# JuliaGaussianProcesses/ApproximateGPs.jl

Hardware: AMD Instinct MI355X
Metric: SVGP ELBO evals/sec at N=1e6, M=1024 (higher is better)
Workload: dtype f64

## Files before the change

### approximategps.jl_amd/csrc/api.hip

```cpp
#include <hip/hip_runtime.h>

#include <algorithm>
#include <functional>
#include <memory>
#include <cmath>
#include <cstdio>
#include <cstddef>
#include <cstdlib>
#include <cstring>
#include <new>
#include <string>
#include <vector>

#include "../../include/svgp_mi355x.h"
#include "ctx.hpp"
#include "kernels.hpp"
#include "knobs.hpp"
#include "lik.hpp"

using namespace svgp;

inline unsigned event_flags(bool timing) {
  static const bool fence = exp_int("SVGP_EVENT_FENCE", 0) == 1;
  return (timing ? 0u : unsigned(hipEventDisableTiming)) | (fence ? 0u : unsigned(hipEventDisableSystemFence));
// ... 136 lines not shown
    m->gh_w.release();
    m->gh_n = 0;
    if (gh > 0) {
      std::vector<double> xs(gh), ws(gh);
      if (gauss_hermite(gh, xs.data(), ws.data()) != SVGP_OK) return fail(ctx, SVGP_INVALID_ARG, "Gauss-Hermite rule failed to converge");
      for (auto& w : ws) w /= 1.7724538509055160273;
      hipError_t e = m->gh_x.alloc(gh * 8);
      if (e == hipSuccess) e = m->gh_w.alloc(gh * 8);
      if (e == hipSuccess) e = hipMemcpy(m->gh_x.p, xs.data(), gh * 8, hipMemcpyHostToDevice);
      if (e == hipSuccess) e = hipMemcpy(m->gh_w.p, ws.data(), gh * 8, hipMemcpyHostToDevice);
      if (e != hipSuccess) {
        m->gh_x.release();
        m->gh_w.release();
        return fail(ctx, e == hipErrorOutOfMemory ? SVGP_OOM : SVGP_HIP_ERROR, std::string("upload of the Gauss-Hermite rule: ") + hipGetErrorString(e));
      }
    }
    m->gh_n = gh;
  }
  HIPC(ctx, hipStreamSynchronize(ctx->stream));
  m->prepared = false;
  return SVGP_OK;
}

KernelParams kparams(const svgp_model* m) {
  KernelParams kp;
  kp.family = m->desc.kernel;
  kp.d = m->d;
  kp.variance = m->desc.variance;
  kp.invl = m->invl.p;
  return kp;
}

inline size_t info_bytes(int64_t Mp) { return (sizeof(int) * size_t(1 + 2 * (Mp / 128)) + 255) / 256 * 256; }
int ensure_overlap(svgp_ctx* ctx, size_t state_doubles);
int enqueue_prep(svgp_ctx* ctx, svgp_model* m, bool overlap = false, const RowHook* hook = nullptr) {
  hipStream_t s = ctx->stream;
  const KernelParams kp = kparams(m);
  HIPC(ctx, hipMemsetAsync(m->info.as<int>(), 0, info_bytes(m->Mp), s));
  launch_scale_inputs(m->dtype, s, m->z_raw.p, m->desc.layout_z, m->d, m->M, m->Mp, m->invl.p, m->zs.p);
  KCHECK(ctx, "scale_inputs");
  if (overlap) {
    launch_pack_q(m->dtype, s, m->Lq_raw.p, m->m_raw.p, m->M, m->Mp, m->U.p, m->mp.p);
    KCHECK(ctx, "pack_q");
    HIPC(ctx, hipEventRecord(ctx->ev_fork, s));
    TREC(ctx, ctx->ev_ov[0], s);
    if (hook && hook->fn) hook->fn(hook->user, -1);
  }
  launch_kuu(m->dtype, s, kp, m->zs.p, m->M, m->Mp, m->desc.jitter, m->L.p);
  KCHECK(ctx, "kuu");
  TREC(ctx, ctx->ev_chol[0], s);
  hipEvent_t rows[16] = {};
  if (overlap) std::copy(std::begin(ctx->ev_row), std::end(ctx->ev_row), rows);
  launch_potrf(m->dtype, s, m->L.p, m->T.p, m->Mp, m->info.as<int>(), reinterpret_cast<unsigned*>(m->info.as<int>() + 1), ctx->num_cus, overlap ? rows : nullptr,
               overlap ? hook : nullptr);
  KCHECK(ctx, "potrf");
  TREC(ctx, ctx->ev_chol[1], s);
  if (overlap) {
    launch_kl_terms(m->dtype, s, m->Lq_raw.p, m->m_raw.p, m->L.p, m->M, m->Mp, m->scal.as<double>());
  } else if (m->desc.parametrization == SVGP_NONCENTERED) {
    launch_pack_q(m->dtype, s, m->Lq_raw.p, m->m_raw.p, m->M, m->Mp, m->U.p, m->mp.p);
    launch_kl_terms(m->dtype, s, m->Lq_raw.p, m->m_raw.p, m->L.p, m->M, m->Mp, m->scal.as<double>());
  } else {
    launch_pad_lower(m->dtype, s, m->Lq_raw.p, m->M, m->Mp, m->B.p);
// ... 77 lines not shown
  int64_t lda = 0;
  bool skip_expect = false;
  const void* mux = nullptr;
};

int enqueue_strips(svgp_ctx* ctx, svgp_model* m, const void* x, int64_t ldx, const void* y, int64_t off, int64_t len,
                   const StripOuts& o) {
  StripPlan plan = strip_plan(m->dtype, m->Mp, len, ctx->num_cus);
  if (plan.concurrent_tail && (o.A || o.C || o.At || o.Ct)) plan = strip_plan_single(m->dtype, m->Mp, len, ctx->num_cus);
  const size_t wb_main = plan.grid ? strip_work_bytes(m->dtype, m->Mp, plan.nt, plan.grid) : 0;
  const size_t wb_tail = plan.nt_tail ? strip_work_bytes(m->dtype, m->Mp, plan.nt_tail, plan.grid_tail) : 0;
  int rc = ensure_scratch(ctx, plan.concurrent_tail ? wb_main : (wb_main > wb_tail ? wb_main : wb_tail), size_t(len));
  if (rc) return rc;
  if (plan.concurrent_tail) {
    rc = ensure_stream2(ctx);
    if (rc) return rc;
    rc = ctx->work2.reserve(ctx, wb_tail, "the concurrent tail's scratch");
    if (rc) return rc;
  }
  StripArgs a{};
  a.T = m->T.p;
  a.U = m->U.p;
  a.zs = m->zs.p;
  a.mp = m->mp.p;
  a.x = x;
  a.work = ctx->work.p;
  a.counter = ctx->counter.as<unsigned>();
  a.mom_mu = ctx->mom_mu();
  a.mom_var = ctx->mom_var();
  a.A_out = o.A;
  a.C_out = o.C;
  a.At_out = o.At;
  a.Ct_out = o.Ct;
  a.lda = o.lda;
  a.ldx = ldx;
  a.off = off;
  a.len = len;
  a.Mp = m->Mp;
  a.M = m->M;
  a.kp = kparams(m);
  a.mean_const = m->desc.mean_const;
  a.mux = o.mux;
  LikParams lp{};
  lp.lik = m->desc.likelihood;
  lp.gh_n = m->gh_n;
  lp.sigma2 = lik_param(m->desc);
// ... 101 lines not shown
  KCHECK(ctx, "strip (segmented: panel)");
  if (I == 0) TREC(ctx, ctx->ev_ov[1], s2);
  if (I == 1 && r.pre) {
    const int rcp = (*r.pre)();
    if (rcp) return rcp;
  }
  return SVGP_OK;
}

void seg_row_hook(void* user, int row) {
  SegRun& r = *static_cast<SegRun*>(user);
  if (r.rc == SVGP_OK) r.rc = seg_enqueue_row(r, row);
}

int seg_prepare_forward(svgp_ctx* ctx, svgp_model* m, const void* x, int64_t ldx, int64_t off, int64_t len, const OverlapPlan& op, SegRun& r) {
  const int nP = int(m->Mp / 128);
  const size_t wb1 = strip_work_bytes(m->dtype, m->Mp, op.nt, int(op.nstrips)), wb = wb1;
  int rc = ctx->work_seg.reserve(ctx, wb, "the segmented strips' scratch");
  if (rc == SVGP_OK) rc = ensure_scratch(ctx, 0, size_t(len));
  if (rc) return rc;
  r.ctx = ctx; r.m = m; r.op = op; r.grad = false; r.nP = nP; r.wb1 = wb1;
  r.split = seg_split_factor(ctx, nP, op.nstrips);
  StripArgs& a = r.a;
  a.T = m->T.p; a.U = m->U.p; a.zs = m->zs.p; a.mp = m->mp.p; a.x = x; a.work = ctx->work_seg.p; a.counter = ctx->counter2.as<unsigned>();
  a.mom_mu = ctx->mom_mu(); a.mom_var = ctx->mom_var();
  a.ldx = ldx; a.off = off; a.len = len; a.Mp = m->Mp; a.M = m->M; a.kp = kparams(m); a.mean_const = m->desc.mean_const;
  a.seg_state = ctx->seg_state.as<double>();
  return SVGP_OK;
}

int seg_finish_forward(svgp_ctx* ctx, svgp_model* m, const void* y, int64_t off, int64_t len, const StripOuts& o, SegRun& r) {
  hipStream_t s = ctx->stream, s2 = ctx->stream2;
  if (r.rc) return r.rc;
  int launches = r.nP + 1;
  if (r.split > 1) {
    StripArgs& a = r.a;
    const int rcs = seg_split_setup(ctx, a, r.split, r.op.nstrips);
    if (rcs) return rcs;
    a.seg_lo = a.seg_hi = r.nP;
    a.seg_flags = kSegLoad | kSegPhase2;
    launch_strip_seg(m->dtype, s2, a, r.op.nt, int(r.op.nstrips) * r.split, r.op.nstrips, false);
    KCHECK(ctx, "strip (segmented: split phase 2)");
    ++launches;
  }
  HIPC(ctx, hipEventRecord(ctx->ev_join, s2));
  HIPC(ctx, hipStreamWaitEvent(s, ctx->ev_join, 0));
  TREC(ctx, ctx->ev[2], s);
// ... 342 lines not shown
  if (!m) return SVGP_OK;
  if (ctx) (void)hipSetDevice(ctx->device);
  delete m;
  return SVGP_OK;
}

int32_t svgp_model_create(svgp_ctx* ctx, const svgp_model_desc* desc, svgp_model** out) {
  if (!ctx) return SVGP_INVALID_ARG;
  if (!out) return fail(ctx, SVGP_INVALID_ARG, "null out pointer");
  *out = nullptr;
  int rc = validate_desc(ctx, desc);
  if (rc) return rc;
  HIPC(ctx, hipSetDevice(ctx->device));
  svgp_model* m = new (std::nothrow) svgp_model();
  if (!m) return SVGP_OOM;
  m->M = desc->M;
  m->Mp = (desc->M + 127) / 128 * 128;
  m->dtype = desc->dtype;
  m->d = desc->d;
  m->es = esize(desc->dtype);
  const size_t es = m->es, M = size_t(m->M), Mp = size_t(m->Mp);
  struct { DevBuf* b; size_t bytes; } allocs[] = {
      {&m->z_raw, M * m->d * es}, {&m->m_raw, M * es},     {&m->Lq_raw, M * M * es}, {&m->invl, size_t(m->d) * es},
      {&m->zs, Mp * m->d * es},   {&m->L, Mp * Mp * es},   {&m->T, Mp * Mp * es},    {&m->U, Mp * Mp * es},
      {&m->mp, Mp * es},          {&m->scal, (8 + Mp) * sizeof(double)},             {&m->info, info_bytes(Mp)},
      {&m->B, desc->parametrization == SVGP_CENTERED ? Mp * Mp * es : 0},
  };
  for (auto& a : allocs)
    if (a.bytes && a.b->alloc(a.bytes) != hipSuccess) {
      svgp_model_free(ctx, m);
      return alloc_failed(ctx, "for model buffers");
    }
  if (hipMemsetAsync(m->T.p, 0, Mp * Mp * es, ctx->stream) != hipSuccess) {
    svgp_model_free(ctx, m);
    return fail(ctx, SVGP_HIP_ERROR, "hipMemsetAsync failed for the model's T buffer");
  }
  rc = upload_params(ctx, m, desc);
  if (rc) {
    svgp_model_free(ctx, m);
    return rc;
  }
  *out = m;
  return SVGP_OK;
}

int32_t svgp_model_update(svgp_ctx* ctx, svgp_model* m, const svgp_model_desc* desc) {
  if (!ctx) return SVGP_INVALID_ARG;
// ... 406 lines not shown
  lp.gh_x = m->gh_x.as<double>();
  lp.gh_w = m->gh_w.as<double>();
  lp.clamp_neg_var = (m->desc.neg_var_policy == SVGP_NEGVAR_CLAMP);
  lp.mean_const = m->desc.mean_const;
  const KernelParams kp = kparams(m);
  double *ext_gmu = nullptr, *ext_gv = nullptr;
  if (gc.ext_gmu) {
    rc = ctx->ext_g.reserve(ctx, 2 * size_t(len) * 8, "the point gradients");
    if (rc) return rc;
    ext_gmu = ctx->ext_g.as<double>();
    ext_gv = ext_gmu + ctx->ext_g.cap / 16;
    HIPC(ctx, hipMemcpyAsync(ext_gmu, gc.ext_gmu, size_t(len) * 8, hipMemcpyHostToDevice, s));
    HIPC(ctx, hipMemcpyAsync(ext_gv, gc.ext_gv, size_t(len) * 8, hipMemcpyHostToDevice, s));
  }
  const bool uniform_w = m->desc.likelihood == SVGP_LIK_GAUSSIAN && !gc.ext_gmu && m->gh_n == 0 && ctx->kn.syrk_uniform;
  static const int early_knob = exp_int("SVGP_SYRK_EARLY", 1);
  const bool syrk_early = gop.on && uniform_w && early_knob != 0;
  if (syrk_early) {
    rc = w->Gmm.reserve(ctx, size_t(std::min<int64_t>(Mp / 128, w->nslices)) * size_t(Mp) * size_t(Mp) * m->es, "the gradient workspace");
    if (rc) return rc;
  }
  auto strip_args = [&](int64_t c0, int64_t clen, LikParams& lpc) -> StripArgs {
    StripArgs a{};
    a.T = m->T.p; a.U = m->U.p; a.zs = m->zs.p; a.mp = m->mp.p; a.x = data->x.p; a.work = ctx->work.p; a.counter = ctx->counter.as<unsigned>();
    a.At_out = w->At.p; a.ldx = data->ldx; a.off = off + c0; a.len = clen; a.Mp = Mp; a.M = M; a.kp = kp;
    a.mean_const = m->desc.mean_const;
    if (gc.mux) a.mux = static_cast<const char*>(gc.mux) + size_t(c0) * es;
    a.mom_mu = ctx->mom_mu(); a.mom_var = ctx->mom_var();
    a.R = w->Rcm.p; a.alpha = w->alpha.p; a.Pt_out = w->Pt.p;
    lpc = lp;
    if (gc.ext_gmu) { lpc.lik = kLikExternal; lpc.gh_x = ext_gmu + c0; lpc.gh_w = ext_gv + c0; }
    return a;
  };
  const void* Bq = centered ? m->B.p : w->Lqp.p;
  auto grad_pre_chain = [&](hipStream_t st) -> int {
    HIPC(ctx, hipMemsetAsync(w->zero_blk.p, 0, w->zero_b, st));
    launch_setvec_f64(st, w->invl_d.as<double>(), m->invl_host.data(), m->d);
    if (!centered) launch_pad_lower(dt, st, m->Lq_raw.p, M, Mp, w->Lqp.p);
    gemm_mm(ctx, w, dt, st, Bq, Bq, Mp, w->G2.p, kMmXUp | kMmYUp);
    launch_sym_from_lower(dt, st, w->G2.p, 1, Mp, 1.0, w->tmp.p);
    KCHECK(ctx, "grad prep (S)");
    return SVGP_OK;
  };
  std::function<int()> seg_pre = [&]() -> int {
    const int rcp = grad_pre_chain(ctx->stream2);
    if (rcp) return rcp;
    HIPC(ctx, hipEventRecord(ctx->ev_S, ctx->stream2));
// ... 614 lines not shown
    const StripPlan plan = strip_plan_single(dt, Mp, clen, ctx->num_cus);
    nt = plan.grid ? plan.nt : plan.nt_tail;
    grid = plan.grid ? plan.grid : plan.grid_tail;
    nstrips = plan.grid ? plan.nstrips : plan.nstrips_tail;
  };
  size_t wb_max = 0;
  const int64_t nchunks = (len + nc - 1) / nc;
  for (int64_t clen : {std::min(len, nc), len - (nchunks - 1) * nc}) {
    int nt, grid; int64_t nstrips;
    chunk_plan(clen, nt, grid, nstrips);
    wb_max = std::max(wb_max, strip_work_bytes(dt, Mp, nt, grid));
  }
  rc = ensure_scratch(ctx, wb_max, size_t(nc));
  if (rc) return rc;
  double* bpart = c->bpart.as<double>();
  double* spart = c->spart.as<double>();
  double* scal = c->scal.as<double>();
  for (int64_t c0 = 0; c0 < len; c0 += nc) {
    const int64_t clen = (len - c0 < nc) ? len - c0 : nc;
    const int64_t ncp = (clen + 127) / 128 * 128;
    int nt, grid; int64_t nstrips;
    chunk_plan(clen, nt, grid, nstrips);
    StripArgs a{};
    a.T = m->T.p; a.zs = m->zs.p; a.x = data->x.p; a.work = ctx->work.p; a.counter = ctx->counter.as<unsigned>();
    a.At_out = w->At.p; a.ldx = data->ldx; a.off = off + c0; a.len = clen; a.Mp = Mp; a.M = M; a.kp = kparams(m);
    a.mom_var = ctx->mom_var();
    HIPC(ctx, hipMemsetAsync(a.counter, 0, sizeof(unsigned), s));
    launch_trsm_point_major(dt, s, a, nt, grid, nstrips);
    KCHECK(ctx, "strip (phase 1, point-major A)");
    const int64_t n16 = (clen + 15) / 16 * 16;
    if (n16 > clen) HIPC(ctx, hipMemsetAsync(static_cast<char*>(w->At.p) + size_t(clen) * size_t(Mp) * es, 0, size_t(n16 - clen) * size_t(Mp) * es, s));
    const int64_t sl = ((ncp + ns_syrk - 1) / ns_syrk + 15) / 16 * 16;
    launch_syrk_uniform(dt, s, w->At.p, 1.0, 1.0, nullptr, 0.0, 1.0, Mp, n16, sl, ns_syrk, w->G1.p, c0 == 0 ? 1 : 0);
    KCHECK(ctx, "syrk (C = A A')");
    launch_collapsed_reduce(dt, s, w->At.p, data->y.p, a.mom_var, Mp, off + c0, clen, m->desc.mean_const, c0 == 0 ? 1 : 0, bpart, spart);
    KCHECK(ctx, "collapsed reduce (b, rr, t)");
  }
  const double sigma2 = m->desc.lik_sigma2;
  int* info_b = c->info_b.as<int>();
  int* info_s = c->info_s.as<int>();
  launch_collapsed_form_b(dt, s, w->G1.p, ns_syrk, Mp, sigma2, bpart, spart, c->Bm.as<double>(), c->cvec.as<double>(), scal);
  HIPC(ctx, hipMemsetAsync(info_b, 0, info_bytes(Mp), s));
  launch_potrf(SVGP_F64, s, c->Bm.p, c->TB.p, Mp, info_b, reinterpret_cast<unsigned*>(info_b + 1), ctx->num_cus);
  launch_trsv2(SVGP_F64, s, c->Bm.p, c->TB.p, Mp, 0, c->cvec.p);
  KCHECK(ctx, "collapsed tail (cholesky(B), c)");
  if (!want_q) {
    launch_collapsed_scal(s, c->Bm.as<double>(), c->cvec.as<double>(), Mp, info_b, nullptr, scal);
// ... 225 lines not shown
```

### approximategps.jl_amd/csrc/kernels.hpp

```cpp
#pragma once
#include <hip/hip_runtime.h>
#include <stdint.h>

namespace svgp {

struct KernelParams {
  int family;
  int d;
  double variance;
  const void* invl;
};

constexpr int kLikExternal = -1;
struct LikParams {
  int lik;
  int gh_n;
  double sigma2;
  double digamma_alpha;
  const double* gh_x;
  const double* gh_w;
  int clamp_neg_var;
  double mean_const;
};

void launch_scale_inputs(int dtype, hipStream_t s, const void* z, int layout, int d, int64_t M, int64_t Mp,
                         const void* invl, void* zs);
void launch_transpose_colvecs(int dtype, hipStream_t s, const void* x_dn, int d, int64_t n, int64_t ldx, void* x_fm);
void launch_kuu(int dtype, hipStream_t s, const KernelParams& kp, const void* zs, int64_t M, int64_t Mp,
                double jitter, void* Kuu);
struct RowHook { void (*fn)(void* user, int row) = nullptr; void* user = nullptr; };
void launch_potrf(int dtype, hipStream_t s, void* A, void* T, int64_t Mp, int* info, unsigned* sync, int num_cus, hipEvent_t* row_events = nullptr,
                  const RowHook* hook = nullptr);
int potrf_max_row_events();
void launch_pack_q(int dtype, hipStream_t s, const void* Lq, const void* m, int64_t M, int64_t Mp, void* U, void* mp);
void launch_kl_terms(int dtype, hipStream_t s, const void* Lq, const void* m, const void* Lk, int64_t M, int64_t Mp,
                     double* scal);
void launch_pack_q_ld(int dtype, hipStream_t s, const void* Lq, int64_t ldq, const void* m, int64_t M, int64_t Mp, void* U,
                       void* mp);
void launch_kl_terms_ld(int dtype, hipStream_t s, const void* Lq, int64_t ldq, const void* m, const void* Lk, int64_t M,
                        int64_t Mp, double* scal);
void launch_trsv2(int dtype, hipStream_t s, const void* L, const void* Tm, int64_t Mp, int trans, void* x);
void launch_trsm_mat(int dtype, hipStream_t s, const void* Tm, int64_t Mp, void* X);
void launch_pad_lower(int dtype, hipStream_t s, const void* Lq, int64_t M, int64_t Mp, void* out);
void launch_shift_vec(int dtype, hipStream_t s, const void* m, double shift, int64_t M, int64_t Mp, void* out);
void launch_shift_sub_vec(int dtype, hipStream_t s, const void* m, double shift, const void* mu, int64_t M, int64_t Mp, void* out);
void launch_extract_lower(int dtype, hipStream_t s, const void* A, int64_t Mp, int64_t M, void* out);

enum : int { kSegPregen = 1, kSegPhase2 = 2, kSegLoad = 4, kSegStore = 8 };
struct StripArgs {
  const void* T;
  const void* U;
  const void* zs;
  const void* mp;
  const void* x;
  unsigned* counter;
  void* work;
  double* mom_mu;
  double* mom_var;
  void* A_out;
  void* C_out;
  void* At_out;
  void* Ct_out;
  int64_t lda;
  int64_t ldx, off, len;
  int64_t Mp, M;
  KernelParams kp;
  double mean_const;
  const void* mux;
  const void* R;
  const void* alpha;
  void* Pt_out;
  int seg_flags;
  int seg_lo, seg_hi;
  double* seg_state;
  int seg_split;
// ... 89 lines not shown
```

### approximategps.jl_amd/csrc/prep.hip

```cpp
#define SVGP_DIAG_TU_PREP
#include "device_common.hpp"
#include "kernels.hpp"
#include "knobs.hpp"

#include <hip/hip_ext.h>
#include <cstdlib>
#include <algorithm>
#include <cmath>
#include <map>
#include <mutex>
#include <vector>

namespace svgp {
namespace {

template <typename T>
__global__ void scale_inputs_kernel(const T* __restrict__ z, int layout, int d, int64_t M, int64_t Mp,
                                    const T* __restrict__ invl, T* __restrict__ zs) {
  const int64_t i = int64_t(blockIdx.x) * blockDim.x + threadIdx.x;
  const int f = blockIdx.y;
  if (i >= Mp) return;
  T v = T(0);
  if (i < M) v = (layout == 1 ? z[int64_t(f) * M + i] : z[i * d + f]) * invl[f];
  zs[int64_t(f) * Mp + i] = v;
}

template <typename T>
__global__ void transpose_colvecs_kernel(const T* __restrict__ x, int d, int64_t n, int64_t ldx, T* __restrict__ out) {
  const int64_t i = int64_t(blockIdx.x) * blockDim.x + threadIdx.x;
  if (i >= n) return;
  for (int f = 0; f < d; ++f) out[int64_t(f) * ldx + i] = x[i * d + f];
}

template <typename T, int DREG>
__global__ void __launch_bounds__(k256) kuu_kernel(KernelParams kp, const T* __restrict__ zs, int64_t M, int64_t Mp, T jitter,
                                                   T* __restrict__ K) {
  constexpr int JB = 16;
  const int64_t i = int64_t(blockIdx.x) * k256 + threadIdx.x;
  const int64_t j0 = int64_t(blockIdx.y) * JB;
  if (i >= Mp || j0 / kNB > (int64_t(blockIdx.x) * k256 + k256 - 1) / kNB) return;
  T zi[DREG > 0 ? DREG : 1];
  if constexpr (DREG > 0) {
#pragma unroll
    for (int f = 0; f < DREG; ++f) zi[f] = (f < kp.d) ? zs[int64_t(f) * Mp + i] : T(0);
  }
  for (int jj = 0; jj < JB; ++jj) {
    const int64_t j = j0 + jj;
// ... 811 lines not shown
  if (!t_inside) {
    hipLaunchKernelGGL((chol_tile_kernel<T, MODE_TRSM, CNT>), dim3((nP * (nP - 1) / 2) * NCH), dim3(k256), lds_tile, s, A, Tm, Mp, -1, 0, info, sync);
    dbg("T panels", s);
  }
}

}

std::string take_note_text() { return take_note(); }

#define SVGP_DISPATCH(dtype, expr_d, expr_f) \
  do {                                       \
    if ((dtype) == 0) { expr_d; } else { expr_f; } \
  } while (0)

void launch_scale_inputs(int dtype, hipStream_t s, const void* z, int layout, int d, int64_t M, int64_t Mp,
                         const void* invl, void* zs) {
  dim3 grid((unsigned)((Mp + 255) / 256), (unsigned)d);
  SVGP_DISPATCH(dtype,
                hipLaunchKernelGGL(scale_inputs_kernel<double>, grid, dim3(256), 0, s, (const double*)z, layout, d, M, Mp, (const double*)invl, (double*)zs),
                hipLaunchKernelGGL(scale_inputs_kernel<float>, grid, dim3(256), 0, s, (const float*)z, layout, d, M, Mp, (const float*)invl, (float*)zs));
}

void launch_transpose_colvecs(int dtype, hipStream_t s, const void* x, int d, int64_t n, int64_t ldx, void* out) {
  dim3 grid((unsigned)((n + 255) / 256));
  SVGP_DISPATCH(dtype,
                hipLaunchKernelGGL(transpose_colvecs_kernel<double>, grid, dim3(256), 0, s, (const double*)x, d, n, ldx, (double*)out),
                hipLaunchKernelGGL(transpose_colvecs_kernel<float>, grid, dim3(256), 0, s, (const float*)x, d, n, ldx, (float*)out));
}

void launch_kuu(int dtype, hipStream_t s, const KernelParams& kp, const void* zs, int64_t M, int64_t Mp, double jitter,
                void* Kuu) {
  dim3 grid((unsigned)((Mp + 255) / 256), (unsigned)(Mp / 16));
  if (kp.d <= 8) {
    SVGP_DISPATCH(dtype,
                  hipLaunchKernelGGL((kuu_kernel<double, 8>), grid, dim3(256), 0, s, kp, (const double*)zs, M, Mp, jitter, (double*)Kuu),
                  hipLaunchKernelGGL((kuu_kernel<float, 8>), grid, dim3(256), 0, s, kp, (const float*)zs, M, Mp, float(jitter), (float*)Kuu));
  } else {
    SVGP_DISPATCH(dtype,
                  hipLaunchKernelGGL((kuu_kernel<double, 0>), grid, dim3(256), 0, s, kp, (const double*)zs, M, Mp, jitter, (double*)Kuu),
                  hipLaunchKernelGGL((kuu_kernel<float, 0>), grid, dim3(256), 0, s, kp, (const float*)zs, M, Mp, float(jitter), (float*)Kuu));
  }
}

void launch_potrf(int dtype, hipStream_t s, void* A, void* T, int64_t Mp, int* info, unsigned* sync, int num_cus, hipEvent_t* row_events,
                  const RowHook* hook) {
// ... 97 lines not shown
```

### approximategps.jl_amd/csrc/strip.hip

```cpp
#define SVGP_DIAG_TU_STRIP
#include "device_common.hpp"
#include "kernels.hpp"
#include "knobs.hpp"
#include "lik.hpp"

#ifndef SVGP_ASYNC
#define SVGP_ASYNC 1
#endif
#ifndef SVGP_TRI
#define SVGP_TRI 3
#endif

#include <cstdlib>
#include <type_traits>

namespace svgp {

namespace {

#ifndef SVGP_PREGEN_EXPTAB
#define SVGP_PREGEN_EXPTAB 1
#endif
template <typename T, int NT, int NTHR, int F, int DL>
__device__ __forceinline__ void pregen_mfma(const T* __restrict__ xs, const T* __restrict__ zs, int d, int64_t Mp, int64_t M,
                                            double variance_d, T* __restrict__ work, const double* __restrict__ exptab = nullptr) {
  constexpr int KS = DL / 4, JT = NT / 16, NW = NTHR / 64;
  constexpr bool XREG = (DL <= 16);
  using M16 = Mfma16<T>;
  using acc_t = typename M16::acc_t;
  const int lane = threadIdx.x & 63, wave = threadIdx.x >> 6, l15 = lane & 15, g = lane >> 4;
  const T variance = T(variance_d);
  const T c1 = (F == KSE) ? T(-0.5) : T(1);
  const T c0 = (F == KSE) ? T(log(variance_d)) : T(0);
  const T ascale = (F == KSE) ? T(1) : T(-2);
  T xb[XREG ? JT : 1][XREG ? KS : 1], xn[JT];
  const T* __restrict__ xl = xs + g * NT + l15;
#pragma unroll
  for (int jt = 0; jt < JT; ++jt) {
    T s = T(0);
#pragma unroll
    for (int q = 0; q < KS; ++q) {
      const T v = xl[(4 * q) * NT + jt * 16];
      if constexpr (XREG) xb[jt][q] = v;
      s = fma(v, v, s);
    }
    s += __shfl_xor(s, 16);
    s += __shfl_xor(s, 32);
    xn[jt] = fma(c1, s, c0);
  }
  for (int kb = wave; kb < int(Mp / 16); kb += NW) {
    const int64_t k0 = int64_t(kb) * 16;
    T za[KS];
    T s = T(0);
#pragma unroll
    for (int q = 0; q < KS; ++q) {
      const int f = 4 * q + g;
      const T v = (f < d) ? zs[int64_t(f) * Mp + k0 + l15] : T(0);
      za[q] = ascale * v;
      s = fma(v, v, s);
    }
    s += __shfl_xor(s, 16);
    s += __shfl_xor(s, 32);
    s *= c1;
    T zn[4];
#pragma unroll
    for (int r = 0; r < 4; ++r) zn[r] = __shfl(s, M16::row(lane, r));
#pragma unroll
    for (int jt = 0; jt < JT; ++jt) {
      acc_t acc;
#pragma unroll
      for (int r = 0; r < 4; ++r) acc[r] = xn[jt] + zn[r];
      if constexpr (XREG) {
#pragma unroll
        for (int q = 0; q < KS; ++q) acc = M16::mma(za[q], xb[jt][q], acc);
      } else {
        acc_t acc2 = {0, 0, 0, 0};
        __builtin_amdgcn_sched_barrier(0);
#pragma unroll
        for (int q = 0; q < KS; q += 2) {
          acc = M16::mma(za[q], xl[(4 * q) * NT + jt * 16], acc);
          acc2 = M16::mma(za[q + 1], xl[(4 * q + 4) * NT + jt * 16], acc2);
        }
#pragma unroll
        for (int r = 0; r < 4; ++r) acc[r] += acc2[r];
      }
#pragma unroll
      for (int r = 0; r < 4; ++r) {
        const int64_t k = k0 + M16::row(lane, r);
        const T v = acc[r];
        T out;
        if constexpr (SVGP_PREGEN_EXPTAB && F == KSE && sizeof(T) == 8) out = T(kexp_tab(double(v > c0 ? c0 : v), exptab));
        else out = (F == KSE) ? kexp(v > c0 ? c0 : v) : kappa<T>(F, v < T(0) ? T(0) : v, variance);
        work[k * NT + jt * 16 + l15] = (k < M) ? out : T(0);
      }
    }
  }
}


template <typename G, typename T, int NT, int NTHR>
__device__ __forceinline__ void store_tile_point_major(const typename G::Acc& acc, T* __restrict__ smem, T* __restrict__ out,
                                                       int64_t c0, int64_t Mp, int row0) {
  constexpr int HC = NT < 64 ? NT : 64, RS = G::NB + (sizeof(T) == 8 ? 4 : 8), VEC = G::VEC, CPR = G::NB / VEC;
  using V = typename G::V;
  static_assert(size_t(HC) * RS * sizeof(T) <= ((SVGP_ASYNC && G::kAsync) ? G::ASYNC_LDS_BYTES : G::LDS_BYTES),
                "the transposition tile must fit the staging buffers");
#pragma unroll
  for (int p = 0; p < NT / HC; ++p) {
#pragma unroll
    for (int j = 0; j < G::NJ; ++j) {
      const int col = G::acc_col(j);
      if (col / HC == p) {
#pragma unroll
        for (int i = 0; i < G::MI; ++i)
#pragma unroll
          for (int r = 0; r < 4; ++r) smem[(col % HC) * RS + G::acc_row(i, r)] = acc.v[i][j][r];
      }
// ... 26 lines not shown
  r.e = expected_loglik_point(lp, mu, v, yv, log(lp.sigma2));
  r.gmu = a * scale;
  r.gv = b * scale;
  r.gs2 = gs2 * scale;
  return r;
}

template <typename T, int NT, int BK, int NTHR, int MINW = 2, int PAD = 16, bool GRAD = false, bool BIGD = false, bool SEG = false>
__global__ void __launch_bounds__(NTHR, MINW) strip_kernel(StripArgs a, int64_t nstrips) {
  using G = TileGemm<T, NT, BK, NTHR, PAD>;
  using Acc = typename G::Acc;
  using QRegs = typename G::QRegs;
  constexpr int NB = G::NB, MI = G::MI, NJ = G::NJ, VEC = G::VEC;

  extern __shared__ __attribute__((aligned(16))) unsigned char smem_raw[];
  T* smem = reinterpret_cast<T*>(smem_raw);
  T* xs = smem;
  const int pre_dl = BIGD ? (a.kp.d <= 32 ? 32 : 64) : (a.kp.d <= 8 ? 8 : a.kp.d <= 16 ? 16 : 0);
  const int dl = pre_dl ? pre_dl : a.kp.d;

  const T* __restrict__ Tm = static_cast<const T*>(a.T);
  const T* __restrict__ U = static_cast<const T*>(a.U);
  const T* __restrict__ zs = static_cast<const T*>(a.zs);
  const T* __restrict__ mp = static_cast<const T*>(a.mp);
  const T* __restrict__ x = static_cast<const T*>(a.x);
  const T* __restrict__ invl = static_cast<const T*>(a.kp.invl);
  const int64_t Mp = a.Mp, M = a.M;
  const int d = a.kp.d, family = a.kp.family;
  const T variance = T(a.kp.variance);
  const int nP = int(Mp / NB);
  T* __restrict__ work = static_cast<T*>(a.work) + int64_t(blockIdx.x) * Mp * NT;
  T* __restrict__ workK = (GRAD && !diag::ablate<256>) ? static_cast<T*>(a.work) + (int64_t(gridDim.x) + blockIdx.x) * Mp * NT : work;
  const int tid = threadIdx.x, lane = tid & 63;
  const typename G::QOff qoff = G::q_offsets(NT);

  __shared__ unsigned next_strip;
#if SVGP_PREGEN_EXPTAB
  __shared__ double s_exptab[64];
  if (sizeof(T) == 8 && threadIdx.x < 64) s_exptab[threadIdx.x] = exp2(double(threadIdx.x) * 0.015625);
  const double* exptab = s_exptab;
#else
  const double* exptab = nullptr;
#endif
  SVGP_SSTAMP_KERNEL_BEGIN();
  [[maybe_unused]] int prio_strips = 0;
  [[maybe_unused]] int part = 0, nsplit = 1;
  if constexpr (SEG) {
    if (a.seg_split > 1) { nsplit = a.seg_split; part = int(blockIdx.x / nstrips); }
  }
  for (int64_t strip = (nsplit > 1) ? int64_t(blockIdx.x % nstrips) : int64_t(blockIdx.x); strip < nstrips;) {
    if constexpr (SEG) {
      work = static_cast<T*>(a.work) + strip * Mp * NT;
      workK = GRAD ? static_cast<T*>(a.work) + (nstrips + strip) * Mp * NT : work;
    }
    SVGP_SSTAMP_STRIP_BEGIN();
    SVGP_SSTAMP(0);
    strip_prio<GRAD && !SEG>(prio_strips++);
    const int64_t c0 = strip * NT;
    if constexpr (SEG) { if (tid == 0) next_strip = unsigned(strip + gridDim.x); }
    else if (tid == 0) next_strip = gridDim.x + atomicAdd(a.counter, 1u);
    const int64_t last = a.off + a.len - 1;
    const bool do_pregen = !SEG || (a.seg_flags & kSegPregen);
    if (do_pregen)
    for (int e = tid; e < dl * NT; e += NTHR) {
      const int f = e / NT, c = e % NT;
      int64_t g = a.off + c0 + c;
      g = g > last ? last : g;
      xs[e] = (f < d) ? x[int64_t(f) * a.ldx + g] * invl[f] : T(0);
    }
    __syncthreads();
    if (do_pregen) {
      auto pregen = [&](auto fam) {
        constexpr int F = decltype(fam)::value;
        using V = typename G::V;
        constexpr int CPR = NT / VEC;
        for (int e = tid; e < int(Mp) * CPR; e += NTHR) {
          const int k = e / CPR, c = (e % CPR) * VEC;
          T r2[VEC];
#pragma unroll
          for (int q = 0; q < VEC; ++q) r2[q] = T(0);
#pragma unroll 8
          for (int f = 0; f < d; ++f) {
            const T zf = zs[int64_t(f) * Mp + k];
            const V xf = *reinterpret_cast<const V*>(xs + f * NT + c);
#pragma unroll
            for (int q = 0; q < VEC; ++q) {
              const T df = xf[q] - zf;
              r2[q] = fma(df, df, r2[q]);
            }
          }
          V out;
#pragma unroll
          for (int q = 0; q < VEC; ++q) out[q] = (k < M) ? kappa<T>(F, r2[q], variance) : T(0);
          *reinterpret_cast<V*>(workK + int64_t(k) * NT + c) = out;
        }
      };
      if constexpr (BIGD) {
        if (pre_dl == 32) {
          if (family == KSE) pregen_mfma<T, NT, NTHR, KSE, 32>(xs, zs, d, Mp, M, a.kp.variance, workK, exptab);
          else if (family == KM32) pregen_mfma<T, NT, NTHR, KM32, 32>(xs, zs, d, Mp, M, a.kp.variance, workK);
          else pregen_mfma<T, NT, NTHR, KM52, 32>(xs, zs, d, Mp, M, a.kp.variance, workK);
        } else {
          if (family == KSE) pregen_mfma<T, NT, NTHR, KSE, 64>(xs, zs, d, Mp, M, a.kp.variance, workK, exptab);
          else if (family == KM32) pregen_mfma<T, NT, NTHR, KM32, 64>(xs, zs, d, Mp, M, a.kp.variance, workK);
          else pregen_mfma<T, NT, NTHR, KM52, 64>(xs, zs, d, Mp, M, a.kp.variance, workK);
        }
      } else if (pre_dl == 8) {
        if (family == KSE) pregen_mfma<T, NT, NTHR, KSE, 8>(xs, zs, d, Mp, M, a.kp.variance, workK, exptab);
        else if (family == KM32) pregen_mfma<T, NT, NTHR, KM32, 8>(xs, zs, d, Mp, M, a.kp.variance, workK);
        else pregen_mfma<T, NT, NTHR, KM52, 8>(xs, zs, d, Mp, M, a.kp.variance, workK);
      } else if (pre_dl == 16) {
        if (family == KSE) pregen_mfma<T, NT, NTHR, KSE, 16>(xs, zs, d, Mp, M, a.kp.variance, workK, exptab);
        else if (family == KM32) pregen_mfma<T, NT, NTHR, KM32, 16>(xs, zs, d, Mp, M, a.kp.variance, workK);
        else pregen_mfma<T, NT, NTHR, KM52, 16>(xs, zs, d, Mp, M, a.kp.variance, workK);
      } else if (family == KSE) pregen(std::integral_constant<int, KSE>{});
      else if (family == KM32) pregen(std::integral_constant<int, KM32>{});
      else pregen(std::integral_constant<int, KM52>{});
      __syncthreads();
    }

    double sA[NJ], sM[NJ], sC[NJ];
#pragma unroll
    for (int j = 0; j < NJ; ++j) sA[j] = sM[j] = sC[j] = 0.0;
    int I_lo = 0, I_hi = nP;
    if constexpr (SEG) {
      I_lo = a.seg_lo;
      I_hi = a.seg_hi;
      if ((a.seg_flags & kSegLoad) && part == 0) {
        const double* __restrict__ st = a.seg_state + (strip * NTHR + tid) * (2 * NJ);
#pragma unroll
        for (int j = 0; j < NJ; ++j) { sA[j] = st[j]; sM[j] = st[NJ + j]; }
      }
    }

    SVGP_SSTAMP(1);
    for (int I = I_lo; I < I_hi; ++I) {
      SVGP_SSTAMP(2 + 3 * I);
// ... 191 lines not shown
      }
      __syncthreads();
      }
    }
    strip = next_strip;
    __syncthreads();
    SVGP_SSTAMP(101);
  }
  SVGP_SSTAMP_KERNEL_END();
}

template <typename T, int NT, int BK, int NTHR, int MINW = 2, int PAD = 16, bool BIGD = false>
__global__ void __launch_bounds__(NTHR, MINW) trsm_pm_kernel(StripArgs a, int64_t nstrips) {
  using G = TileGemm<T, NT, BK, NTHR, PAD>;
  using Acc = typename G::Acc;
  using QRegs = typename G::QRegs;
  constexpr int NB = G::NB, MI = G::MI, NJ = G::NJ;

  extern __shared__ __attribute__((aligned(16))) unsigned char smem_raw[];
  T* smem = reinterpret_cast<T*>(smem_raw);
  T* xs = smem;
  const int pre_dl = BIGD ? (a.kp.d <= 32 ? 32 : 64) : (a.kp.d <= 8 ? 8 : 16);
  const T* __restrict__ Tm = static_cast<const T*>(a.T);
  const T* __restrict__ zs = static_cast<const T*>(a.zs);
  const T* __restrict__ x = static_cast<const T*>(a.x);
  const T* __restrict__ invl = static_cast<const T*>(a.kp.invl);
  const int64_t Mp = a.Mp, M = a.M;
  const int d = a.kp.d, family = a.kp.family;
  const int nP = int(Mp / NB);
  T* __restrict__ work = static_cast<T*>(a.work) + int64_t(blockIdx.x) * Mp * NT;
  const int tid = threadIdx.x, lane = tid & 63;
  [[maybe_unused]] const typename G::QOff qoff = G::q_offsets(NT);

  __shared__ unsigned next_strip;
#if SVGP_PREGEN_EXPTAB
  __shared__ double s_exptab[64];
  if (sizeof(T) == 8 && threadIdx.x < 64) s_exptab[threadIdx.x] = exp2(double(threadIdx.x) * 0.015625);
  const double* exptab = s_exptab;
#else
  const double* exptab = nullptr;
#endif
  for (int64_t strip = blockIdx.x; strip < nstrips;) {
    const int64_t c0 = strip * NT;
    if (tid == 0) next_strip = gridDim.x + atomicAdd(a.counter, 1u);
    const int64_t last = a.off + a.len - 1;
    for (int e = tid; e < pre_dl * NT; e += NTHR) {
      const int f = e / NT, c = e % NT;
      int64_t g = a.off + c0 + c;
      g = g > last ? last : g;
      xs[e] = (f < d) ? x[int64_t(f) * a.ldx + g] * invl[f] : T(0);
    }
    __syncthreads();
    if constexpr (BIGD) {
      if (pre_dl == 32) {
        if (family == KSE) pregen_mfma<T, NT, NTHR, KSE, 32>(xs, zs, d, Mp, M, a.kp.variance, work, exptab);
        else if (family == KM32) pregen_mfma<T, NT, NTHR, KM32, 32>(xs, zs, d, Mp, M, a.kp.variance, work);
        else pregen_mfma<T, NT, NTHR, KM52, 32>(xs, zs, d, Mp, M, a.kp.variance, work);
      } else {
        if (family == KSE) pregen_mfma<T, NT, NTHR, KSE, 64>(xs, zs, d, Mp, M, a.kp.variance, work, exptab);
        else if (family == KM32) pregen_mfma<T, NT, NTHR, KM32, 64>(xs, zs, d, Mp, M, a.kp.variance, work);
        else pregen_mfma<T, NT, NTHR, KM52, 64>(xs, zs, d, Mp, M, a.kp.variance, work);
      }
    } else if (pre_dl == 8) {
      if (family == KSE) pregen_mfma<T, NT, NTHR, KSE, 8>(xs, zs, d, Mp, M, a.kp.variance, work, exptab);
      else if (family == KM32) pregen_mfma<T, NT, NTHR, KM32, 8>(xs, zs, d, Mp, M, a.kp.variance, work);
      else pregen_mfma<T, NT, NTHR, KM52, 8>(xs, zs, d, Mp, M, a.kp.variance, work);
    } else {
      if (family == KSE) pregen_mfma<T, NT, NTHR, KSE, 16>(xs, zs, d, Mp, M, a.kp.variance, work, exptab);
      else if (family == KM32) pregen_mfma<T, NT, NTHR, KM32, 16>(xs, zs, d, Mp, M, a.kp.variance, work);
      else pregen_mfma<T, NT, NTHR, KM52, 16>(xs, zs, d, Mp, M, a.kp.variance, work);
    }
    __syncthreads();

    double sA[NJ];
#pragma unroll
    for (int j = 0; j < NJ; ++j) sA[j] = 0.0;
    for (int I = 0; I < nP; ++I) {
      Acc acc;
      acc.zero();
      if constexpr (SVGP_ASYNC && G::kAsync) {
        auto qsrc = [&](int t) { return work + int64_t(t) * BK * NT; };
        G::template loop_tri_async<(SVGP_TRI & 1) ? 1 : 0>(acc, Tm + int64_t(I) * NB, Mp, (I + 1) * (NB / BK), qsrc, smem);
      } else {
        auto qload = [&](int t, QRegs& r) { G::load_q(r, work + int64_t(t) * BK * NT, qoff); };
        G::template loop_tri<(BK == 16 && (SVGP_TRI & 1)) ? 1 : 0>(acc, Tm + int64_t(I) * NB, Mp, (I + 1) * (NB / BK), qload, smem);
      }
#pragma unroll
      for (int i = 0; i < MI; ++i) {
#pragma unroll
        for (int r = 0; r < 4; ++r) {
          const int row = I * NB + G::acc_row(i, r);
#pragma unroll
          for (int j = 0; j < NJ; ++j) {
// ... 668 lines not shown
```

Measured before the change: 29.70.

## Precompute per-lane inducing-point image once and software-prefetch it in pregen

Adds a prep kernel that packs the scaled inducing points into a per-lane, MFMA-ready image (scaled coordinates plus half squared norms), computed once per model preparation. The strip pregen loop then loads this image with vector loads and prefetches the next block, instead of re-gathering zs and re-running the norm reduction and shuffles for every strip. It also interleaves pairs of column-tile MFMA chains, and restructures the x staging loop so invl is hoisted per feature. The costs are extra model memory, one more prep launch, and higher register pressure from the prefetch buffer.

```diff
diff --git a/approximategps.jl_amd/csrc/api.hip b/approximategps.jl_amd/csrc/api.hip
--- a/approximategps.jl_amd/csrc/api.hip
+++ b/approximategps.jl_amd/csrc/api.hip
@@ -182,6 +182,8 @@
   return SVGP_OK;
 }
 
+inline void* zimg_of(const svgp_model* m) { return static_cast<char*>(m->zs.p) + size_t(m->Mp) * m->d * m->es; }
+
 KernelParams kparams(const svgp_model* m) {
   KernelParams kp;
   kp.family = m->desc.kernel;
@@ -199,6 +201,8 @@
   HIPC(ctx, hipMemsetAsync(m->info.as<int>(), 0, info_bytes(m->Mp), s));
   launch_scale_inputs(m->dtype, s, m->z_raw.p, m->desc.layout_z, m->d, m->M, m->Mp, m->invl.p, m->zs.p);
   KCHECK(ctx, "scale_inputs");
+  launch_pregen_image(m->dtype, s, kp, m->zs.p, m->Mp, zimg_of(m));
+  KCHECK(ctx, "pregen_image");
   if (overlap) {
     launch_pack_q(m->dtype, s, m->Lq_raw.p, m->m_raw.p, m->M, m->Mp, m->U.p, m->mp.p);
     KCHECK(ctx, "pack_q");
@@ -322,6 +326,7 @@
   a.T = m->T.p;
   a.U = m->U.p;
   a.zs = m->zs.p;
+  a.zimg = zimg_of(m);
   a.mp = m->mp.p;
   a.x = x;
   a.work = ctx->work.p;
@@ -469,7 +474,7 @@
   r.ctx = ctx; r.m = m; r.op = op; r.grad = false; r.nP = nP; r.wb1 = wb1;
   r.split = seg_split_factor(ctx, nP, op.nstrips);
   StripArgs& a = r.a;
-  a.T = m->T.p; a.U = m->U.p; a.zs = m->zs.p; a.mp = m->mp.p; a.x = x; a.work = ctx->work_seg.p; a.counter = ctx->counter2.as<unsigned>();
+  a.T = m->T.p; a.U = m->U.p; a.zs = m->zs.p; a.zimg = zimg_of(m); a.mp = m->mp.p; a.x = x; a.work = ctx->work_seg.p; a.counter = ctx->counter2.as<unsigned>();
   a.mom_mu = ctx->mom_mu(); a.mom_var = ctx->mom_var();
   a.ldx = ldx; a.off = off; a.len = len; a.Mp = m->Mp; a.M = m->M; a.kp = kparams(m); a.mean_const = m->desc.mean_const;
   a.seg_state = ctx->seg_state.as<double>();
@@ -858,7 +863,7 @@
   const size_t es = m->es, M = size_t(m->M), Mp = size_t(m->Mp);
   struct { DevBuf* b; size_t bytes; } allocs[] = {
       {&m->z_raw, M * m->d * es}, {&m->m_raw, M * es},     {&m->Lq_raw, M * M * es}, {&m->invl, size_t(m->d) * es},
-      {&m->zs, Mp * m->d * es},   {&m->L, Mp * Mp * es},   {&m->T, Mp * Mp * es},    {&m->U, Mp * Mp * es},
+      {&m->zs, (Mp * m->d + pregen_image_elems(m->d, m->Mp)) * es},   {&m->L, Mp * Mp * es},   {&m->T, Mp * Mp * es},    {&m->U, Mp * Mp * es},
       {&m->mp, Mp * es},          {&m->scal, (8 + Mp) * sizeof(double)},             {&m->info, info_bytes(Mp)},
       {&m->B, desc->parametrization == SVGP_CENTERED ? Mp * Mp * es : 0},
   };
@@ -1311,7 +1316,7 @@
   }
   auto strip_args = [&](int64_t c0, int64_t clen, LikParams& lpc) -> StripArgs {
     StripArgs a{};
-    a.T = m->T.p; a.U = m->U.p; a.zs = m->zs.p; a.mp = m->mp.p; a.x = data->x.p; a.work = ctx->work.p; a.counter = ctx->counter.as<unsigned>();
+    a.T = m->T.p; a.U = m->U.p; a.zs = m->zs.p; a.zimg = zimg_of(m); a.mp = m->mp.p; a.x = data->x.p; a.work = ctx->work.p; a.counter = ctx->counter.as<unsigned>();
     a.At_out = w->At.p; a.ldx = data->ldx; a.off = off + c0; a.len = clen; a.Mp = Mp; a.M = M; a.kp = kp;
     a.mean_const = m->desc.mean_const;
     if (gc.mux) a.mux = static_cast<const char*>(gc.mux) + size_t(c0) * es;
@@ -1972,7 +1977,7 @@
     int nt, grid; int64_t nstrips;
     chunk_plan(clen, nt, grid, nstrips);
     StripArgs a{};
-    a.T = m->T.p; a.zs = m->zs.p; a.x = data->x.p; a.work = ctx->work.p; a.counter = ctx->counter.as<unsigned>();
+    a.T = m->T.p; a.zs = m->zs.p; a.zimg = zimg_of(m); a.x = data->x.p; a.work = ctx->work.p; a.counter = ctx->counter.as<unsigned>();
     a.At_out = w->At.p; a.ldx = data->ldx; a.off = off + c0; a.len = clen; a.Mp = Mp; a.M = M; a.kp = kparams(m);
     a.mom_var = ctx->mom_var();
     HIPC(ctx, hipMemsetAsync(a.counter, 0, sizeof(unsigned), s));
diff --git a/approximategps.jl_amd/csrc/kernels.hpp b/approximategps.jl_amd/csrc/kernels.hpp
--- a/approximategps.jl_amd/csrc/kernels.hpp
+++ b/approximategps.jl_amd/csrc/kernels.hpp
@@ -25,6 +25,9 @@
 
 void launch_scale_inputs(int dtype, hipStream_t s, const void* z, int layout, int d, int64_t M, int64_t Mp,
                          const void* invl, void* zs);
+inline int pregen_dl(int d) { return d <= 8 ? 8 : d <= 16 ? 16 : d <= 32 ? 32 : 64; }
+inline size_t pregen_image_elems(int d, int64_t Mp) { return size_t(Mp / 16) * 64 * size_t(pregen_dl(d) / 4 + 4); }
+void launch_pregen_image(int dtype, hipStream_t s, const KernelParams& kp, const void* zs, int64_t Mp, void* img);
 void launch_transpose_colvecs(int dtype, hipStream_t s, const void* x_dn, int d, int64_t n, int64_t ldx, void* x_fm);
 void launch_kuu(int dtype, hipStream_t s, const KernelParams& kp, const void* zs, int64_t M, int64_t Mp,
                 double jitter, void* Kuu);
@@ -51,6 +54,7 @@
   const void* T;
   const void* U;
   const void* zs;
+  const void* zimg;
   const void* mp;
   const void* x;
   unsigned* counter;
diff --git a/approximategps.jl_amd/csrc/prep.hip b/approximategps.jl_amd/csrc/prep.hip
--- a/approximategps.jl_amd/csrc/prep.hip
+++ b/approximategps.jl_amd/csrc/prep.hip
@@ -23,6 +23,31 @@
   T v = T(0);
   if (i < M) v = (layout == 1 ? z[int64_t(f) * M + i] : z[i * d + f]) * invl[f];
   zs[int64_t(f) * Mp + i] = v;
+}
+
+template <typename T, int DL>
+__global__ void __launch_bounds__(k256) pregen_image_kernel(int family, int d, int64_t Mp, const T* __restrict__ zs, T* __restrict__ img) {
+  constexpr int KS = DL / 4, E = KS + 4;
+  using M16 = Mfma16<T>;
+  const int lane = threadIdx.x & 63, l15 = lane & 15, g = lane >> 4;
+  const int64_t kb = int64_t(blockIdx.x) * (k256 / 64) + (threadIdx.x >> 6);
+  if (kb >= Mp / 16) return;
+  const T c1 = (family == KSE) ? T(-0.5) : T(1);
+  const T ascale = (family == KSE) ? T(1) : T(-2);
+  T* __restrict__ out = img + (kb * 64 + lane) * E;
+  T s = T(0);
+#pragma unroll
+  for (int q = 0; q < KS; ++q) {
+    const int f = 4 * q + g;
+    const T v = (f < d) ? zs[int64_t(f) * Mp + kb * 16 + l15] : T(0);
+    out[q] = ascale * v;
+    s = fma(v, v, s);
+  }
+  s += __shfl_xor(s, 16);
+  s += __shfl_xor(s, 32);
+  s *= c1;
+#pragma unroll
+  for (int r = 0; r < 4; ++r) out[KS + r] = __shfl(s, M16::row(lane, r));
 }
 
 template <typename T>
@@ -880,6 +905,24 @@
                 hipLaunchKernelGGL(scale_inputs_kernel<float>, grid, dim3(256), 0, s, (const float*)z, layout, d, M, Mp, (const float*)invl, (float*)zs));
 }
 
+namespace {
+template <typename T>
+void launch_pregen_image_t(hipStream_t s, const KernelParams& kp, const T* zs, int64_t Mp, T* img) {
+  const dim3 grid((unsigned)(Mp / 16 / (k256 / 64)));
+  switch (pregen_dl(kp.d)) {
+    case 8: hipLaunchKernelGGL((pregen_image_kernel<T, 8>), grid, dim3(k256), 0, s, kp.family, kp.d, Mp, zs, img); break;
+    case 16: hipLaunchKernelGGL((pregen_image_kernel<T, 16>), grid, dim3(k256), 0, s, kp.family, kp.d, Mp, zs, img); break;
+    case 32: hipLaunchKernelGGL((pregen_image_kernel<T, 32>), grid, dim3(k256), 0, s, kp.family, kp.d, Mp, zs, img); break;
+    default: hipLaunchKernelGGL((pregen_image_kernel<T, 64>), grid, dim3(k256), 0, s, kp.family, kp.d, Mp, zs, img); break;
+  }
+}
+}
+
+void launch_pregen_image(int dtype, hipStream_t s, const KernelParams& kp, const void* zs, int64_t Mp, void* img) {
+  SVGP_DISPATCH(dtype, launch_pregen_image_t<double>(s, kp, (const double*)zs, Mp, (double*)img),
+                launch_pregen_image_t<float>(s, kp, (const float*)zs, Mp, (float*)img));
+}
+
 void launch_transpose_colvecs(int dtype, hipStream_t s, const void* x, int d, int64_t n, int64_t ldx, void* out) {
   dim3 grid((unsigned)((n + 255) / 256));
   SVGP_DISPATCH(dtype,
diff --git a/approximategps.jl_amd/csrc/strip.hip b/approximategps.jl_amd/csrc/strip.hip
--- a/approximategps.jl_amd/csrc/strip.hip
+++ b/approximategps.jl_amd/csrc/strip.hip
@@ -22,19 +22,31 @@
 #define SVGP_PREGEN_EXPTAB 1
 #endif
 template <typename T, int NT, int NTHR, int F, int DL>
-__device__ __forceinline__ void pregen_mfma(const T* __restrict__ xs, const T* __restrict__ zs, int d, int64_t Mp, int64_t M,
+__device__ __forceinline__ void pregen_mfma(const T* __restrict__ xs, const T* __restrict__ zimg, int64_t Mp, int64_t M,
                                             double variance_d, T* __restrict__ work, const double* __restrict__ exptab = nullptr) {
-  constexpr int KS = DL / 4, JT = NT / 16, NW = NTHR / 64;
+  constexpr int KS = DL / 4, JT = NT / 16, NW = NTHR / 64, E = KS + 4;
+  constexpr int VW = (E % int(16 / sizeof(T)) == 0) ? int(16 / sizeof(T)) : int(8 / sizeof(T));
   constexpr bool XREG = (DL <= 16);
+  static_assert(JT % 2 == 0 && E % VW == 0, "column tiles go in pairs; a lane's image is whole vectors");
   using M16 = Mfma16<T>;
   using acc_t = typename M16::acc_t;
+  using ZV = T __attribute__((ext_vector_type(VW)));
+  struct ZBlk { ZV v[E / VW]; };
   const int lane = threadIdx.x & 63, wave = threadIdx.x >> 6, l15 = lane & 15, g = lane >> 4;
   const T variance = T(variance_d);
   const T c1 = (F == KSE) ? T(-0.5) : T(1);
   const T c0 = (F == KSE) ? T(log(variance_d)) : T(0);
-  const T ascale = (F == KSE) ? T(1) : T(-2);
   T xb[XREG ? JT : 1][XREG ? KS : 1], xn[JT];
   const T* __restrict__ xl = xs + g * NT + l15;
+  const int nkb = int(Mp / 16);
+  auto zload = [&](int kb) {
+    const ZV* __restrict__ p = reinterpret_cast<const ZV*>(zimg + (int64_t(kb) * 64 + lane) * E);
+    ZBlk b;
+#pragma unroll
+    for (int i = 0; i < E / VW; ++i) b.v[i] = p[i];
+    return b;
+  };
+  ZBlk nxt = zload(wave);
 #pragma unroll
   for (int jt = 0; jt < JT; ++jt) {
     T s = T(0);
@@ -48,42 +60,34 @@
     s += __shfl_xor(s, 32);
     xn[jt] = fma(c1, s, c0);
   }
-  for (int kb = wave; kb < int(Mp / 16); kb += NW) {
+#pragma unroll
+  for (int i = 0; i < E / VW; ++i) asm volatile("" : "+v"(nxt.v[i]));
+  for (int kb = wave; kb < nkb; kb += NW) {
     const int64_t k0 = int64_t(kb) * 16;
-    T za[KS];
-    T s = T(0);
-#pragma unroll
-    for (int q = 0; q < KS; ++q) {
-      const int f = 4 * q + g;
-      const T v = (f < d) ? zs[int64_t(f) * Mp + k0 + l15] : T(0);
-      za[q] = ascale * v;
-      s = fma(v, v, s);
-    }
-    s += __shfl_xor(s, 16);
-    s += __shfl_xor(s, 32);
-    s *= c1;
-    T zn[4];
-#pragma unroll
-    for (int r = 0; r < 4; ++r) zn[r] = __shfl(s, M16::row(lane, r));
-#pragma unroll
-    for (int jt = 0; jt < JT; ++jt) {
+    const ZBlk cur = nxt;
+    nxt = zload(kb + NW < nkb ? kb + NW : kb);
+    auto zv = [&](int e) { return cur.v[e / VW][e % VW]; };
+    auto chain = [&](int jt) {
       acc_t acc;
 #pragma unroll
-      for (int r = 0; r < 4; ++r) acc[r] = xn[jt] + zn[r];
+      for (int r = 0; r < 4; ++r) acc[r] = xn[jt] + zv(KS + r);
       if constexpr (XREG) {
 #pragma unroll
-        for (int q = 0; q < KS; ++q) acc = M16::mma(za[q], xb[jt][q], acc);
+        for (int q = 0; q < KS; ++q) acc = M16::mma(zv(q), xb[jt][q], acc);
       } else {
         acc_t acc2 = {0, 0, 0, 0};
         __builtin_amdgcn_sched_barrier(0);
 #pragma unroll
         for (int q = 0; q < KS; q += 2) {
-          acc = M16::mma(za[q], xl[(4 * q) * NT + jt * 16], acc);
-          acc2 = M16::mma(za[q + 1], xl[(4 * q + 4) * NT + jt * 16], acc2);
+          acc = M16::mma(zv(q), xl[(4 * q) * NT + jt * 16], acc);
+          acc2 = M16::mma(zv(q + 1), xl[(4 * q + 4) * NT + jt * 16], acc2);
         }
 #pragma unroll
         for (int r = 0; r < 4; ++r) acc[r] += acc2[r];
       }
+      return acc;
+    };
+    auto emit = [&](int jt, const acc_t& acc) {
 #pragma unroll
       for (int r = 0; r < 4; ++r) {
         const int64_t k = k0 + M16::row(lane, r);
@@ -93,6 +97,12 @@
         else out = (F == KSE) ? kexp(v > c0 ? c0 : v) : kappa<T>(F, v < T(0) ? T(0) : v, variance);
         work[k * NT + jt * 16 + l15] = (k < M) ? out : T(0);
       }
+    };
+#pragma unroll
+    for (int jt = 0; jt < JT; jt += 2) {
+      const acc_t a0 = chain(jt), a1 = chain(jt + 1);
+      emit(jt, a0);
+      emit(jt + 1, a1);
     }
   }
 }
@@ -165,6 +175,7 @@
   const T* __restrict__ Tm = static_cast<const T*>(a.T);
   const T* __restrict__ U = static_cast<const T*>(a.U);
   const T* __restrict__ zs = static_cast<const T*>(a.zs);
+  const T* __restrict__ zimg = static_cast<const T*>(a.zimg);
   const T* __restrict__ mp = static_cast<const T*>(a.mp);
   const T* __restrict__ x = static_cast<const T*>(a.x);
   const T* __restrict__ invl = static_cast<const T*>(a.kp.invl);
@@ -205,11 +216,13 @@
     const int64_t last = a.off + a.len - 1;
     const bool do_pregen = !SEG || (a.seg_flags & kSegPregen);
     if (do_pregen)
-    for (int e = tid; e < dl * NT; e += NTHR) {
-      const int f = e / NT, c = e % NT;
-      int64_t g = a.off + c0 + c;
-      g = g > last ? last : g;
-      xs[e] = (f < d) ? x[int64_t(f) * a.ldx + g] * invl[f] : T(0);
+    for (int f = tid >> 6; f < dl; f += NTHR / 64) {
+      const T il = (f < d) ? invl[f] : T(0);
+      for (int c = lane; c < NT; c += 64) {
+        int64_t g = a.off + c0 + c;
+        g = g > last ? last : g;
+        xs[f * NT + c] = (f < d) ? x[int64_t(f) * a.ldx + g] * il : T(0);
+      }
     }
     __syncthreads();
     if (do_pregen) {
@@ -240,22 +253,22 @@
       };
       if constexpr (BIGD) {
         if (pre_dl == 32) {
-          if (family == KSE) pregen_mfma<T, NT, NTHR, KSE, 32>(xs, zs, d, Mp, M, a.kp.variance, workK, exptab);
-          else if (family == KM32) pregen_mfma<T, NT, NTHR, KM32, 32>(xs, zs, d, Mp, M, a.kp.variance, workK);
-          else pregen_mfma<T, NT, NTHR, KM52, 32>(xs, zs, d, Mp, M, a.kp.variance, workK);
+          if (family == KSE) pregen_mfma<T, NT, NTHR, KSE, 32>(xs, zimg, Mp, M, a.kp.variance, workK, exptab);
+          else if (family == KM32) pregen_mfma<T, NT, NTHR, KM32, 32>(xs, zimg, Mp, M, a.kp.variance, workK);
+          else pregen_mfma<T, NT, NTHR, KM52, 32>(xs, zimg, Mp, M, a.kp.variance, workK);
         } else {
-          if (family == KSE) pregen_mfma<T, NT, NTHR, KSE, 64>(xs, zs, d, Mp, M, a.kp.variance, workK, exptab);
-          else if (family == KM32) pregen_mfma<T, NT, NTHR, KM32, 64>(xs, zs, d, Mp, M, a.kp.variance, workK);
-          else pregen_mfma<T, NT, NTHR, KM52, 64>(xs, zs, d, Mp, M, a.kp.variance, workK);
+          if (family == KSE) pregen_mfma<T, NT, NTHR, KSE, 64>(xs, zimg, Mp, M, a.kp.variance, workK, exptab);
+          else if (family == KM32) pregen_mfma<T, NT, NTHR, KM32, 64>(xs, zimg, Mp, M, a.kp.variance, workK);
+          else pregen_mfma<T, NT, NTHR, KM52, 64>(xs, zimg, Mp, M, a.kp.variance, workK);
         }
       } else if (pre_dl == 8) {
-        if (family == KSE) pregen_mfma<T, NT, NTHR, KSE, 8>(xs, zs, d, Mp, M, a.kp.variance, workK, exptab);
-        else if (family == KM32) pregen_mfma<T, NT, NTHR, KM32, 8>(xs, zs, d, Mp, M, a.kp.variance, workK);
-        else pregen_mfma<T, NT, NTHR, KM52, 8>(xs, zs, d, Mp, M, a.kp.variance, workK);
+        if (family == KSE) pregen_mfma<T, NT, NTHR, KSE, 8>(xs, zimg, Mp, M, a.kp.variance, workK, exptab);
+        else if (family == KM32) pregen_mfma<T, NT, NTHR, KM32, 8>(xs, zimg, Mp, M, a.kp.variance, workK);
+        else pregen_mfma<T, NT, NTHR, KM52, 8>(xs, zimg, Mp, M, a.kp.variance, workK);
       } else if (pre_dl == 16) {
-        if (family == KSE) pregen_mfma<T, NT, NTHR, KSE, 16>(xs, zs, d, Mp, M, a.kp.variance, workK, exptab);
-        else if (family == KM32) pregen_mfma<T, NT, NTHR, KM32, 16>(xs, zs, d, Mp, M, a.kp.variance, workK);
-        else pregen_mfma<T, NT, NTHR, KM52, 16>(xs, zs, d, Mp, M, a.kp.variance, workK);
+        if (family == KSE) pregen_mfma<T, NT, NTHR, KSE, 16>(xs, zimg, Mp, M, a.kp.variance, workK, exptab);
+        else if (family == KM32) pregen_mfma<T, NT, NTHR, KM32, 16>(xs, zimg, Mp, M, a.kp.variance, workK);
+        else pregen_mfma<T, NT, NTHR, KM52, 16>(xs, zimg, Mp, M, a.kp.variance, workK);
       } else if (family == KSE) pregen(std::integral_constant<int, KSE>{});
       else if (family == KM32) pregen(std::integral_constant<int, KM32>{});
       else pregen(std::integral_constant<int, KM52>{});
@@ -493,7 +506,7 @@
   T* xs = smem;
   const int pre_dl = BIGD ? (a.kp.d <= 32 ? 32 : 64) : (a.kp.d <= 8 ? 8 : 16);
   const T* __restrict__ Tm = static_cast<const T*>(a.T);
-  const T* __restrict__ zs = static_cast<const T*>(a.zs);
+  const T* __restrict__ zimg = static_cast<const T*>(a.zimg);
   const T* __restrict__ x = static_cast<const T*>(a.x);
   const T* __restrict__ invl = static_cast<const T*>(a.kp.invl);
   const int64_t Mp = a.Mp, M = a.M;
@@ -515,31 +528,33 @@
     const int64_t c0 = strip * NT;
     if (tid == 0) next_strip = gridDim.x + atomicAdd(a.counter, 1u);
     const int64_t last = a.off + a.len - 1;
-    for (int e = tid; e < pre_dl * NT; e += NTHR) {
-      const int f = e / NT, c = e % NT;
-      int64_t g = a.off + c0 + c;
-      g = g > last ? last : g;
-      xs[e] = (f < d) ? x[int64_t(f) * a.ldx + g] * invl[f] : T(0);
+    for (int f = tid >> 6; f < pre_dl; f += 4) {
+      const T il = (f < d) ? invl[f] : T(0);
+      for (int c = lane; c < NT; c += 64) {
+        int64_t g = a.off + c0 + c;
+        g = g > last ? last : g;
+        xs[f * NT + c] = (f < d) ? x[int64_t(f) * a.ldx + g] * il : T(0);
+      }
     }
     __syncthreads();
     if constexpr (BIGD) {
       if (pre_dl == 32) {
-        if (family == KSE) pregen_mfma<T, NT, NTHR, KSE, 32>(xs, zs, d, Mp, M, a.kp.variance, work, exptab);
-        else if (family == KM32) pregen_mfma<T, NT, NTHR, KM32, 32>(xs, zs, d, Mp, M, a.kp.variance, work);
-        else pregen_mfma<T, NT, NTHR, KM52, 32>(xs, zs, d, Mp, M, a.kp.variance, work);
+        if (family == KSE) pregen_mfma<T, NT, NTHR, KSE, 32>(xs, zimg, Mp, M, a.kp.variance, work, exptab);
+        else if (family == KM32) pregen_mfma<T, NT, NTHR, KM32, 32>(xs, zimg, Mp, M, a.kp.variance, work);
+        else pregen_mfma<T, NT, NTHR, KM52, 32>(xs, zimg, Mp, M, a.kp.variance, work);
       } else {
-        if (family == KSE) pregen_mfma<T, NT, NTHR, KSE, 64>(xs, zs, d, Mp, M, a.kp.variance, work, exptab);
-        else if (family == KM32) pregen_mfma<T, NT, NTHR, KM32, 64>(xs, zs, d, Mp, M, a.kp.variance, work);
-        else pregen_mfma<T, NT, NTHR, KM52, 64>(xs, zs, d, Mp, M, a.kp.variance, work);
+        if (family == KSE) pregen_mfma<T, NT, NTHR, KSE, 64>(xs, zimg, Mp, M, a.kp.variance, work, exptab);
+        else if (family == KM32) pregen_mfma<T, NT, NTHR, KM32, 64>(xs, zimg, Mp, M, a.kp.variance, work);
+        else pregen_mfma<T, NT, NTHR, KM52, 64>(xs, zimg, Mp, M, a.kp.variance, work);
       }
     } else if (pre_dl == 8) {
-      if (family == KSE) pregen_mfma<T, NT, NTHR, KSE, 8>(xs, zs, d, Mp, M, a.kp.variance, work, exptab);
-      else if (family == KM32) pregen_mfma<T, NT, NTHR, KM32, 8>(xs, zs, d, Mp, M, a.kp.variance, work);
-      else pregen_mfma<T, NT, NTHR, KM52, 8>(xs, zs, d, Mp, M, a.kp.variance, work);
+      if (family == KSE) pregen_mfma<T, NT, NTHR, KSE, 8>(xs, zimg, Mp, M, a.kp.variance, work, exptab);
+      else if (family == KM32) pregen_mfma<T, NT, NTHR, KM32, 8>(xs, zimg, Mp, M, a.kp.variance, work);
+      else pregen_mfma<T, NT, NTHR, KM52, 8>(xs, zimg, Mp, M, a.kp.variance, work);
     } else {
-      if (family == KSE) pregen_mfma<T, NT, NTHR, KSE, 16>(xs, zs, d, Mp, M, a.kp.variance, work, exptab);
-      else if (family == KM32) pregen_mfma<T, NT, NTHR, KM32, 16>(xs, zs, d, Mp, M, a.kp.variance, work);
-      else pregen_mfma<T, NT, NTHR, KM52, 16>(xs, zs, d, Mp, M, a.kp.variance, work);
+      if (family == KSE) pregen_mfma<T, NT, NTHR, KSE, 16>(xs, zimg, Mp, M, a.kp.variance, work, exptab);
+      else if (family == KM32) pregen_mfma<T, NT, NTHR, KM32, 16>(xs, zimg, Mp, M, a.kp.variance, work);
+      else pregen_mfma<T, NT, NTHR, KM52, 16>(xs, zimg, Mp, M, a.kp.variance, work);
     }
     __syncthreads();
 
```

Result: no change. 29.77 (median of 6 runs) (+0.2%).
